# pandegroup/openmm

Hardware: NVIDIA H100
Metric: ns/day (higher is better)
Workload: dtype f32

## Files before the change

### include/b200md.h

```cpp
#ifndef B200MD_H_
#define B200MD_H_

#include <stdint.h>

#ifdef __cplusplus
extern "C" {
#endif

typedef struct b200md_ctx b200md_ctx;

#define B200MD_NB_NOCUTOFF            0
#define B200MD_NB_CUTOFF_NONPERIODIC  1
#define B200MD_NB_CUTOFF_PERIODIC     2
#define B200MD_NB_EWALD               3
#define B200MD_NB_PME                 4
#define B200MD_NB_LJPME               5

#define B200MD_TERM_BONDS      1
#define B200MD_TERM_ANGLES     2
#define B200MD_TERM_TORSIONS   4
#define B200MD_TERM_NB_DIRECT  8
#define B200MD_TERM_NB_RECIP   16
#define B200MD_TERM_RB_TORSIONS 32
#define B200MD_TERM_CMAP       64
// ... 72 lines not shown

int b200md_compute(b200md_ctx* ctx, int terms, int want_forces, double* energy);
int b200md_compute_groups(b200md_ctx* ctx, int terms, unsigned int bonded_group_mask, int want_forces, double* energy);

int b200md_set_integrator(b200md_ctx* ctx, int kind, double dt, double temperature, double friction,
                          int seed, double constraint_tol);
int b200md_step(b200md_ctx* ctx, int nsteps);
int b200md_integrate_only(b200md_ctx* ctx);
int b200md_kinetic_energy(b200md_ctx* ctx, double* ke);
int b200md_apply_constraints(b200md_ctx* ctx, double tol);
int b200md_apply_velocity_constraints(b200md_ctx* ctx, double tol);
int b200md_synchronize(b200md_ctx* ctx);

int b200md_comm_unique_id(void* id128);
int b200md_ownership_probe(int natoms, const double* mass, int ncon, const int* p1, const int* p2, const double* distance,
                           int world, int* atom_lo, int* unit_lo);
int b200md_comm_init(b200md_ctx* ctx, int rank, int world, const void* id128);

typedef struct b200md_stats {
    int64_t natoms, padded_atoms, num_blocks;
    int64_t num_tiles;
    int64_t num_mask_tiles;
    int64_t list_builds;
    int64_t force_evals;
    int64_t kernel_launches;
    int64_t pairs_in_cutoff;
    int     pme_grid[3];
    double  ewald_alpha;
    int     overflow;
    int64_t graph_instantiations;
} b200md_stats;
int b200md_get_stats(b200md_ctx* ctx, b200md_stats* out);
int b200md_time_phase(b200md_ctx* ctx, int phase, int reps, double* ms_mean);
int b200md_fft3d_r2c(int device, int nx, int ny, int nz, const float* in, float* out);
int b200md_fft3d_c2r(int device, int nx, int ny, int nz, const float* in, float* out);
void* b200md_cuda_stream(b200md_ctx* ctx);

int b200md_pme_create(b200md_ctx** out, int device, int natoms, int nx, int ny, int nz, double alpha);
int b200md_pme_exec(b200md_ctx* ctx, const float* posq, const double box[9], int include_energy, float* force4, double* energy);

#ifdef __cplusplus
}
#endif
#endif
```

### openmm_b200/_lib.py

```python
import ctypes as C
import os

_HERE = os.path.dirname(os.path.abspath(__file__))
LIB_PATH = os.environ.get("B200MD_LIB", os.path.join(_HERE, "libb200md.so"))


class NonbondedDesc(C.Structure):
    _fields_ = [("method", C.c_int), ("cutoff", C.c_double), ("use_switch", C.c_int), ("switch_distance", C.c_double),
                ("rf_dielectric", C.c_double), ("ewald_alpha", C.c_double), ("grid", C.c_int*3),
                ("dispersion_coefficient", C.c_double), ("exceptions_periodic", C.c_int)]


class Stats(C.Structure):
    _fields_ = [("natoms", C.c_int64), ("padded_atoms", C.c_int64), ("num_blocks", C.c_int64), ("num_tiles", C.c_int64),
                ("num_mask_tiles", C.c_int64), ("list_builds", C.c_int64), ("force_evals", C.c_int64),
                ("kernel_launches", C.c_int64), ("pairs_in_cutoff", C.c_int64), ("pme_grid", C.c_int*3),
                ("ewald_alpha", C.c_double), ("overflow", C.c_int),
                ("graph_instantiations", C.c_int64)]


_P = C.c_void_p
_D = C.POINTER(C.c_double)
_I = C.POINTER(C.c_int)
_F = C.POINTER(C.c_float)
# ... 23 lines not shown
    "b200md_update_nonbonded_params": (C.c_int, [_P, _D, _D, _D, C.c_int, _D, _D, _D, C.c_double]),
    "b200md_update_bonded_params": (C.c_int, [_P, C.c_int, C.c_int, _D, _D, _I]),
    "b200md_update_rb_torsion_params": (C.c_int, [_P, C.c_int, _D]),
    "b200md_update_cmap_params": (C.c_int, [_P, C.c_int, _I, _D, C.c_int, _I]),
    "b200md_set_box": (C.c_int, [_P, _D, _D, _D]),
    "b200md_get_box": (C.c_int, [_P, _D, _D, _D]),
    "b200md_set_barostat_molecules": (C.c_int, [_P, C.c_int, _I, _I]),
    "b200md_scale_coordinates": (C.c_int, [_P, C.c_double, C.c_double, C.c_double]),
    "b200md_restore_coordinates": (C.c_int, [_P]),
    "b200md_set_positions": (C.c_int, [_P, _D]),
    "b200md_get_positions": (C.c_int, [_P, _D]),
    "b200md_set_velocities": (C.c_int, [_P, _D]),
    "b200md_get_velocities": (C.c_int, [_P, _D]),
    "b200md_get_forces": (C.c_int, [_P, _D]),
    "b200md_set_time": (C.c_int, [_P, C.c_double]),
    "b200md_get_time": (C.c_double, [_P]),
    "b200md_get_step_count": (C.c_int64, [_P]),
    "b200md_checkpoint_save": (C.c_int64, [_P, _P, C.c_int64]),
    "b200md_checkpoint_load": (C.c_int, [_P, _P, C.c_int64]),
    "b200md_compute": (C.c_int, [_P, C.c_int, C.c_int, _D]),
    "b200md_compute_groups": (C.c_int, [_P, C.c_int, C.c_uint, C.c_int, _D]),
    "b200md_set_integrator": (C.c_int, [_P, C.c_int, C.c_double, C.c_double, C.c_double, C.c_int, C.c_double]),
    "b200md_step": (C.c_int, [_P, C.c_int]),
    "b200md_integrate_only": (C.c_int, [_P]),
    "b200md_kinetic_energy": (C.c_int, [_P, _D]),
    "b200md_apply_constraints": (C.c_int, [_P, C.c_double]),
    "b200md_apply_velocity_constraints": (C.c_int, [_P, C.c_double]),
    "b200md_synchronize": (C.c_int, [_P]),
    "b200md_comm_unique_id": (C.c_int, [_P]),
    "b200md_ownership_probe": (C.c_int, [C.c_int, _D, C.c_int, _I, _I, _D, C.c_int, _I, _I]),
    "b200md_comm_init": (C.c_int, [_P, C.c_int, C.c_int, _P]),
    "b200md_get_stats": (C.c_int, [_P, C.POINTER(Stats)]),
    "b200md_time_phase": (C.c_int, [_P, C.c_int, C.c_int, _D]),
    "b200md_fft3d_r2c": (C.c_int, [C.c_int, C.c_int, C.c_int, C.c_int, _F, _F]),
    "b200md_fft3d_c2r": (C.c_int, [C.c_int, C.c_int, C.c_int, C.c_int, _F, _F]),
    "b200md_pme_create": (C.c_int, [C.POINTER(_P), C.c_int, C.c_int, C.c_int, C.c_int, C.c_int, C.c_double]),
    "b200md_pme_exec": (C.c_int, [_P, _F, _D, C.c_int, _F, _D]),
    "b200md_cuda_stream": (_P, [_P]),
}

_lib = None


def load():
    global _lib
    if _lib is None:
        if not os.path.exists(LIB_PATH):
            raise RuntimeError("libb200md.so is missing (%s): build it with `python -c 'import __graft_entry__ as g; g.build()'`. "
                               "openmm_b200 has no CPU fallback." % LIB_PATH)
        lib = C.CDLL(LIB_PATH, mode=C.RTLD_GLOBAL)
        for name, (res, args) in SIGNATURES.items():
            fn = getattr(lib, name)
            fn.restype = res
            fn.argtypes = args
        _lib = lib
    return _lib
```

### openmm_b200/csrc/engine.cu

```cuda
#include "engine.h"
#include "../../include/b200md.h"
#include <stdexcept>
#include <algorithm>
#include <cmath>
#include <cstring>
#include <cstdlib>
#include <map>
#include <set>
#include <dlfcn.h>
#include <thread>

static std::string g_create_error;

template <class T> struct DevBuf {
    T* p = nullptr; size_t n = 0; bool owned = true;
    void attach(void* ptr, size_t count) { free(); p = (T*) ptr; n = count; owned = false; }
    void alloc(size_t count) {
        if (!owned) { if (count > n) throw std::runtime_error("window buffer too small"); return; }
        free(); n = count; if (count) CUDA_CHECK(cudaMalloc(&p, count*sizeof(T)));
    }
    void upload(const std::vector<T>& v) { if (v.size() > n) alloc(v.size()); if (!v.empty()) CUDA_CHECK(cudaMemcpy(p, v.data(), v.size()*sizeof(T), cudaMemcpyHostToDevice)); }
    void zero() { if (n) CUDA_CHECK(cudaMemset(p, 0, n*sizeof(T))); }
    void free() { if (p && owned) cudaFree(p); p = nullptr; n = 0; owned = true; }
    ~DevBuf() { free(); }
// ... 308 lines not shown
}

static void cell_order(const int nc[3], std::vector<int>& rank) {
    const int sx = (nc[0] + 1)/2, sy = (nc[1] + 1)/2, sz = (nc[2] + 1)/2;
    rank.assign((size_t) nc[0]*nc[1]*nc[2], 0);
    int r = 0;
    for (int ix = 0; ix < sx; ix++)
        for (int jy = 0; jy < sy; jy++) {
            const int iy = (ix & 1) ? sy-1-jy : jy;
            for (int kz = 0; kz < sz; kz++) {
                const int iz = ((ix*sy + jy) & 1) ? sz-1-kz : kz;
                for (int a = 0; a < 2; a++) for (int b = 0; b < 2; b++) for (int c = 0; c < 2; c++) {
                    const int x = 2*ix + a, y = 2*iy + b, z = 2*iz + c;
                    if (x < nc[0] && y < nc[1] && z < nc[2]) rank[((size_t) x*nc[1] + y)*nc[2] + z] = r++;
                }
            }
        }
}

static void setup_cells(b200md_ctx* c) {
    int nc[3] = {1, 1, 1};
    if (c->nb.box.periodic) {
        const double vol = c->boxA[0]*c->boxB[1]*c->boxC[2];
        const double density = c->natoms/vol;
        double edge = std::cbrt(4.0/density);
        const double L[3] = {c->boxA[0], c->boxB[1], c->boxC[2]};
        for (int d = 0; d < 3; d++) nc[d] = std::max(1, std::min(128, (int) std::floor(L[d]/edge)));
    }
    const int ncells = nc[0]*nc[1]*nc[2];
    if (ncells != c->nb.ncells || nc[0] != c->nb.ncell[0] || nc[1] != c->nb.ncell[1] || nc[2] != c->nb.ncell[2]) {
        std::vector<int> rank;
        cell_order(nc, rank);
        c->cellRank.upload(rank);
        c->cellCount.alloc(ncells + 1); c->cellCount.zero();
        c->cellFill.alloc(ncells); c->cellFill.zero();
        c->nb.ncells = ncells;
        for (int d = 0; d < 3; d++) c->nb.ncell[d] = nc[d];
        c->nb.cellRank = c->cellRank.p; c->nb.cellCount = c->cellCount.p; c->nb.cellFill = c->cellFill.p;
    }
}

static void invalidate_graph(b200md_ctx* c) { c->graphValid = false; c->multiValid = false; }

static void apply_box(b200md_ctx* c) {
    BoxDev& b = c->nb.box;
    const int m = c->nbdesc.method;
    b.periodic = (m == B200MD_NB_CUTOFF_PERIODIC || m == B200MD_NB_PME) ? 1 : 0;
    if (c->haveBox) {
        b.ax = (float) c->boxA[0]; b.bx = (float) c->boxB[0]; b.by = (float) c->boxB[1];
        b.cx = (float) c->boxC[0]; b.cy = (float) c->boxC[1]; b.cz = (float) c->boxC[2];
        b.invAx = (float) (1.0/c->boxA[0]); b.invBy = (float) (1.0/c->boxB[1]); b.invCz = (float) (1.0/c->boxC[2]);
        b.dax = c->boxA[0]; b.dby = c->boxB[1]; b.dcz = c->boxC[2];
        b.triclinic = (c->boxB[0] != 0 || c->boxC[0] != 0 || c->boxC[1] != 0) ? 1 : 0;
        const double det = c->boxA[0]*c->boxB[1]*c->boxC[2];
        const double s = 1.0/det;
        double* R = b.recip;
        R[0] = c->boxB[1]*c->boxC[2]*s; R[1] = 0; R[2] = 0;
        R[3] = -c->boxB[0]*c->boxC[2]*s; R[4] = c->boxA[0]*c->boxC[2]*s; R[5] = 0;
        R[6] = (c->boxB[0]*c->boxC[1] - c->boxB[1]*c->boxC[0])*s; R[7] = -c->boxA[0]*c->boxC[1]*s; R[8] = c->boxA[0]*c->boxB[1]*s;
        b.volume = det;
    }
    else {
        require(!b.periodic, "periodic nonbonded method needs box vectors (b200md_set_box)");
        b.ax = b.by = b.cz = 1.f; b.bx = b.cx = b.cy = 0.f; b.invAx = b.invBy = b.invCz = 1.f; b.triclinic = 0; b.dax = b.dby = b.dcz = 1;
        for (int i = 0; i < 9; i++) b.recip[i] = 0; b.volume = 1;
    }
    if (b.periodic) {
// ... 1417 lines not shown
    c->forceEvals++;
    c->hforce.resize((size_t) 3*c->npad);
    double he[B200MD_NUM_ENERGY] = {0};
    CUDA_CHECK(cudaMemcpyAsync(c->hforce.data(), c->force.p, sizeof(long long)*3*c->npad, cudaMemcpyDeviceToHost, c->stream));
    if (include_energy) CUDA_CHECK(cudaMemcpyAsync(he, c->energy.p, sizeof(he), cudaMemcpyDeviceToHost, c->stream));
    CUDA_CHECK(cudaStreamSynchronize(c->stream));
    const double s = 1.0/B200MD_FORCE_SCALE;
    for (int i = 0; i < c->natoms; i++)
        for (int k = 0; k < 3; k++) force4[4*i+k] = (float) (s*(double) c->hforce[(size_t) k*c->npad + i]);
    if (energy) *energy = include_energy ? he[EN_RECIP] : 0.0;
    API_END(ctx)
}

extern "C" int b200md_get_stats(b200md_ctx* ctx, b200md_stats* out) {
    API_BEGIN(ctx)
    memset(out, 0, sizeof(*out));
    out->natoms = ctx->natoms; out->padded_atoms = ctx->npad; out->num_blocks = ctx->nblocks;
    if (ctx->finalized) {
        launch_count_pairs(ctx->nb, ctx->stream);
        int h[16], lc[2*LC_STRIDE];
        CUDA_CHECK(cudaMemcpyAsync(h, ctx->counters.p, sizeof(int)*16, cudaMemcpyDeviceToHost, ctx->stream));
        CUDA_CHECK(cudaMemcpyAsync(lc, ctx->listCounters.p, sizeof(lc), cudaMemcpyDeviceToHost, ctx->stream));
        CUDA_CHECK(cudaStreamSynchronize(ctx->stream));
        const int* cur = lc + LC_STRIDE*(h[CT_CUR] & 1);
        int masks = 0;
        for (int r = 0; r < TILE_REGIONS; r++) masks += cur[LC_MASKS + r];
        out->num_tiles = cur[LC_USED]; out->num_mask_tiles = masks; out->overflow = h[CT_OVERFLOW]; out->list_builds = h[CT_BUILDS]; out->pairs_in_cutoff = h[CT_PAIRS];
    }
    out->force_evals = ctx->forceEvals; out->kernel_launches = ctx->kernelLaunches; out->graph_instantiations = ctx->graphInstantiations;
    out->pme_grid[0] = ctx->pme.nx; out->pme_grid[1] = ctx->pme.ny; out->pme_grid[2] = ctx->pme.nz; out->ewald_alpha = ctx->pme.alpha;
    API_END(ctx)
}

extern "C" int b200md_time_phase(b200md_ctx* ctx, int phase, int reps, double* ms_mean) {
    API_BEGIN(ctx)
    require(ctx->finalized, "time_phase before finalize");
    b200md_ctx* c = ctx;
    prepare_list(c);
    c->stepStateValid = false;
    cudaStream_t s = c->stream;
    const NbDev nbv = role_nb(c);
    CommDev local{}; local.world = 1;
    cudaEvent_t e0, e1;
    CUDA_CHECK(cudaEventCreate(&e0)); CUDA_CHECK(cudaEventCreate(&e1));
    const int one = 1;
    double total = 0;
    DevBuf<float4> savePos, saveVel, saveCorr; DevBuf<double4> saveVelD; unsigned long long saveStep = 0;
    auto restoreState = [&]() {
        CUDA_CHECK(cudaMemcpyAsync(c->posq.p, savePos.p, sizeof(float4)*c->npad, cudaMemcpyDeviceToDevice, s));
        CUDA_CHECK(cudaMemcpyAsync(c->velm.p, saveVel.p, sizeof(float4)*c->npad, cudaMemcpyDeviceToDevice, s));
        if (c->mixed()) {
            CUDA_CHECK(cudaMemcpyAsync(c->posqCorr.p, saveCorr.p, sizeof(float4)*c->npad, cudaMemcpyDeviceToDevice, s));
            CUDA_CHECK(cudaMemcpyAsync(c->velmD.p, saveVelD.p, sizeof(double4)*c->npad, cudaMemcpyDeviceToDevice, s));
        }
    };
    if (phase == 4) {
        require(c->haveIntegrator, "time_phase(integrate) before set_integrator");
        savePos.alloc(c->npad); saveVel.alloc(c->npad);
        CUDA_CHECK(cudaMemcpyAsync(savePos.p, c->posq.p, sizeof(float4)*c->npad, cudaMemcpyDeviceToDevice, s));
        CUDA_CHECK(cudaMemcpyAsync(saveVel.p, c->velm.p, sizeof(float4)*c->npad, cudaMemcpyDeviceToDevice, s));
        if (c->mixed()) {
            saveCorr.alloc(c->npad); saveVelD.alloc(c->npad);
            CUDA_CHECK(cudaMemcpyAsync(saveCorr.p, c->posqCorr.p, sizeof(float4)*c->npad, cudaMemcpyDeviceToDevice, s));
            CUDA_CHECK(cudaMemcpyAsync(saveVelD.p, c->velmD.p, sizeof(double4)*c->npad, cudaMemcpyDeviceToDevice, s));
        }
        CUDA_CHECK(cudaMemcpyAsync(&saveStep, c->stepCounter.p, sizeof(saveStep), cudaMemcpyDeviceToHost, s));
// ... 70 lines not shown
```

### openmm_b200/csrc/engine.h

```cpp
#pragma once
#include <cuda_runtime.h>
#include <stdint.h>
#include <stdexcept>
#include <string>
#include <vector>

#define B200MD_TILE 32
#define B200MD_PME_ORDER 5
#define B200MD_FORCE_SCALE 4294967296.0
#define B200MD_ONE_4PI_EPS0 138.93545764438198
#define B200MD_BOLTZ 0.00831446261815324
#define B200MD_MAX_RADIX 16
#define B200MD_MAX_FFT_STAGES 8

#define CUDA_CHECK(x) do { cudaError_t e_ = (x); if (e_ != cudaSuccess) throw std::runtime_error(std::string(#x) + ": " + cudaGetErrorString(e_)); } while (0)

template <typename... P, typename... A>
inline void launch_high(void (*kernel)(P...), dim3 grid, dim3 block, size_t smem, cudaStream_t s, A... args) {
    static const int hi = [] { int lo = 0, h = 0; cudaDeviceGetStreamPriorityRange(&lo, &h); return h; }();
    cudaLaunchAttribute at[1];
    at[0].id = cudaLaunchAttributePriority;
    at[0].val.priority = hi;
    cudaLaunchConfig_t cfg = {};
    cfg.gridDim = grid; cfg.blockDim = block; cfg.dynamicSmemBytes = smem; cfg.stream = s;
// ... 16 lines not shown
typedef double2 real2;
#else
typedef float real;
typedef float2 real2;
#endif

struct FftPlanDev {
    int n;
    int nstages;
    int radix[B200MD_MAX_FFT_STAGES];
    const real2* tw;
};

struct ListDev {
    float4* sposq;
    float2* ssigeps;
    float4* swrap;
    int* sorig;
    float4* blockCenter;
    float4* blockHalf;
    float4* superCenter;
    float4* superHalf;
    int* tileI;
    int* tileJ;
    int* tileMask;
    unsigned int* maskPool;
    int* lc;
};
#define TILE_REGIONS 32
enum { LC_TILES = 0, LC_MASKS = TILE_REGIONS, LC_MAXHALF = 2*TILE_REGIONS, LC_USED = 2*TILE_REGIONS + 1, LC_STRIDE = 128 };

enum { CT_PAIRSTART = 0,
       CT_REBUILD = 2, CT_OVERFLOW = 3, CT_BUILDS = 4, CT_PAIRS = 5, CT_CUR = 10, CT_CURSOR = 14,
       CT_BTDONE = 7, CT_BAR = 9, CT_BAREXIT = 15 };

struct NbDev {
    BoxDev box;
    int natoms, npad, nblocks;
    int method;
    int useSwitch;
    float cutoff, cutoff2, paddedCutoff2, switchDist;
    float alpha;
    float krf, crf;
    float dispDummy;
    float4* posq;
    float4* velm;
    float4* posqCorr;
    double4* velmD;
    float2* sigeps;
    const double* chargeD;
    const double2* sigepsD;
    long long* force;
    double* energy;
    ListDev list[2];
    int* sortedOf;
    float4* refPos;
    int ncell[3];
    int ncells;
    const int* cellRank;
    int* cellCount;
    int* cellFill;
    int* atomCell;
    int* tmpSorted;
    float4* atomShift;
    int maxTiles;
    int* counters;
    const int* exclStart;
// ... 306 lines not shown
```

### openmm_b200/csrc/nonbonded.cu

```cuda
#include "engine.h"
#include "../../include/b200md.h"
#include <algorithm>

#define FULL 0xffffffffu

__device__ __forceinline__ float3 min_image(float3 d, const BoxDev& b) {
    if (b.triclinic) {
        float s = floorf(d.z*b.invCz + 0.5f);
        d.x -= s*b.cx; d.y -= s*b.cy; d.z -= s*b.cz;
        s = floorf(d.y*b.invBy + 0.5f);
        d.x -= s*b.bx; d.y -= s*b.by;
        s = floorf(d.x*b.invAx + 0.5f);
        d.x -= s*b.ax;
    }
    else {
        d.x -= b.ax*rintf(d.x*b.invAx);
        d.y -= b.by*rintf(d.y*b.invBy);
        d.z -= b.cz*rintf(d.z*b.invCz);
    }
    return d;
}

__device__ __forceinline__ float box_dist2(float3 d, float hx, float hy, float hz, const BoxDev& b, bool periodic) {
    if (periodic) d = min_image(d, b);
    if (!periodic || !b.triclinic) {
        const float dx = fmaxf(0.f, fabsf(d.x) - hx), dy = fmaxf(0.f, fabsf(d.y) - hy), dz = fmaxf(0.f, fabsf(d.z) - hz);
        return dx*dx + dy*dy + dz*dz;
    }
    float best = 3e38f;
    for (int sz = -1; sz <= 1; sz++)
        for (int sy = -1; sy <= 1; sy++)
            for (int sx = -1; sx <= 1; sx++) {
                const float x = d.x + sx*b.ax + sy*b.bx + sz*b.cx;
                const float y = d.y + sy*b.by + sz*b.cy;
                const float z = d.z + sz*b.cz;
                const float dx = fmaxf(0.f, fabsf(x) - hx), dy = fmaxf(0.f, fabsf(y) - hy), dz = fmaxf(0.f, fabsf(z) - hz);
                best = fminf(best, dx*dx + dy*dy + dz*dz);
            }
    return best;
}

__global__ void __launch_bounds__(256) k_check_gather(NbDev nb, CommDev cd) {
    comm_wait(cd, CH_POS, cd.world > 1 ? *cd.posNeed : 0ull);
    const int s = blockIdx.x*blockDim.x + threadIdx.x;
    const ListDev& L = nb.list[nb.counters[CT_CUR] & 1];
    if (s == 0) { nb.counters[CT_CURSOR] = 0; nb.counters[CT_PAIRSTART] = 0; }
    if (s < nb.natoms) {
        const float4 p = nb.posq[s];
        const float4 r = nb.refPos[s];
        const float dx = p.x-r.x, dy = p.y-r.y, dz = p.z-r.z;
        const float d2 = dx*dx + dy*dy + dz*dz;
        if (!(d2 <= nb.halfPad2))
            nb.counters[CT_REBUILD] = 1;
    }
    if (s < nb.npad) {
        int a = L.sorig[s];
        if (a < 0 || a >= nb.natoms) a = L.sorig[nb.natoms-1];
        a = min(max(a, 0), nb.natoms-1);
        float4 p = nb.posq[a];
        if (s >= nb.natoms) p.w = 0.f;
        L.sposq[s] = p;
    }
}

__device__ __forceinline__ void wrap_molecule(const NbDev& nb, int m) {
    const int begin = nb.molStart[m], end = nb.molStart[m+1];
    const float4 p = nb.posq[nb.molAtoms[begin]];
    const double* R = nb.box.recip;
    const double px = p.x - nb.origin[0], py = p.y - nb.origin[1], pz = p.z - nb.origin[2];
    const double f[3] = {px*R[0] + py*R[3] + pz*R[6], px*R[1] + py*R[4] + pz*R[7], px*R[2] + py*R[5] + pz*R[8]};
    int k[3];
    bool move = false;
    for (int d = 0; d < 3; d++) {
        const double w = floor(f[d]);
        k[d] = (w >= 2.0 || w <= -2.0) ? (int) w : 0;
        move |= (k[d] != 0);
    }
    if (!move) return;
    const BoxDev& b = nb.box;
    const double sx = -(k[0]*(double) b.dax + k[1]*(double) b.bx + k[2]*(double) b.cx);
    const double sy = -(k[1]*(double) b.dby + k[2]*(double) b.cy);
    const double sz = -(k[2]*(double) b.dcz);
    for (int t = begin; t < end; t++) {
        const int a = nb.molAtoms[t];
        if (nb.posqCorr) {
            const double4 q = load_pos<double>(nb, a);
            store_pos<double>(nb, a, q.x + sx, q.y + sy, q.z + sz);
        }
        else {
            const float4 q = nb.posq[a];
            nb.posq[a] = make_float4((float) ((double) q.x + sx), (float) ((double) q.y + sy), (float) ((double) q.z + sz), q.w);
        }
        nb.cellOffset[a] += k[0]; nb.cellOffset[a + nb.npad] += k[1]; nb.cellOffset[a + 2*nb.npad] += k[2];
    }
}

__device__ __forceinline__ void bin_atom(const NbDev& nb, int a) {
    float4 p = nb.posq[a];
    int key = 0;
    float4 shift = make_float4(0, 0, 0, 0);
    if (nb.box.periodic) {
        const double* R = nb.box.recip;
        double f[3];
        const double px = p.x - nb.origin[0], py = p.y - nb.origin[1], pz = p.z - nb.origin[2];
        f[0] = px*R[0] + py*R[3] + pz*R[6];
        f[1] = px*R[1] + py*R[4] + pz*R[7];
        f[2] = px*R[2] + py*R[5] + pz*R[8];
        int c[3];
        float fl[3];
        for (int d = 0; d < 3; d++) {
            double w = floor(f[d]);
            fl[d] = (float) w;
            double fr = f[d] - w;
            int ci = (int) (fr*nb.ncell[d]);
            c[d] = min(max(ci, 0), nb.ncell[d]-1);
        }
        shift.x = -(fl[0]*nb.box.ax + fl[1]*nb.box.bx + fl[2]*nb.box.cx);
        shift.y = -(fl[1]*nb.box.by + fl[2]*nb.box.cy);
        shift.z = -(fl[2]*nb.box.cz);
        key = nb.cellRank[(c[0]*nb.ncell[1] + c[1])*nb.ncell[2] + c[2]];
    }
    else
        key = 0;
    nb.atomCell[a] = key;
    nb.atomShift[a] = shift;
    atomicAdd(&nb.cellCount[key], 1);
}

__device__ void scan_cells_block(const NbDev& nb, int* partial) {
    int n = nb.ncells;
    int per = (n + blockDim.x - 1)/blockDim.x;
    int begin = threadIdx.x*per, end = min(begin+per, n);
    int sum = 0;
    for (int i = begin; i < end; i++) sum += nb.cellCount[i];
    partial[threadIdx.x] = sum;
    __syncthreads();
    for (int off = 1; off < blockDim.x; off <<= 1) {
        int v = (threadIdx.x >= off) ? partial[threadIdx.x-off] : 0;
        __syncthreads();
        partial[threadIdx.x] += v;
        __syncthreads();
    }
    int run = partial[threadIdx.x] - sum;
    for (int i = begin; i < end; i++) {
        int c = nb.cellCount[i];
        nb.cellCount[i] = run;
        run += c;
    }
    if (threadIdx.x == 0) nb.cellCount[n] = nb.natoms;
}

__device__ __forceinline__ void fill_atom(const NbDev& nb, int a) {
    int key = nb.atomCell[a];
    int slot = nb.cellCount[key] + atomicAdd(&nb.cellFill[key], 1);
    nb.tmpSorted[slot] = a;
}

__device__ __forceinline__ void finalize_slot(const NbDev& nb, const ListDev& L, int s) {
    if (s < nb.natoms) {
        int a = s;
        if (nb.box.periodic) {
            a = nb.tmpSorted[s];
            const int key = nb.atomCell[a];
            const int begin = nb.cellCount[key], end = nb.cellCount[key+1];
            int rank = 0;
            for (int t = begin; t < end; t++) rank += (nb.tmpSorted[t] < a);
            s = begin + rank;
        }
        float4 p = nb.posq[a];
        float4 sh = nb.atomShift[a];
        L.sorig[s] = a;
        nb.sortedOf[a] = s;
        L.swrap[s] = make_float4(p.x+sh.x, p.y+sh.y, p.z+sh.z, p.w);
        L.sposq[s] = p;
        L.ssigeps[s] = nb.sigeps[a];
        nb.refPos[a] = p;
        if (s == 0) L.lc[LC_MAXHALF] = 0;
    }
    else {
        L.sorig[s] = -1;
        L.ssigeps[s] = make_float2(0, 0);
    }
}

__device__ __forceinline__ void grid_barrier(const NbDev& nb, int target) {
    __syncthreads();
    if (threadIdx.x == 0) {
        __threadfence();
        atomicAdd(&nb.counters[CT_BAR], 1);
        long spins = 0;
        while (*((volatile int*) &nb.counters[CT_BAR]) < target) {
            __nanosleep(32);
            if (++spins > (1L << 23)) { nb.counters[CT_OVERFLOW] = 2; break; }
        }
        __threadfence();
    }
    __syncthreads();
}

__device__ void list_prep_phases(const NbDev& nb, const ListDev& L, int* partial) {
    const int G = gridDim.x;
    const int gtid = blockIdx.x*blockDim.x + threadIdx.x, gthreads = G*blockDim.x;
    const int lane = threadIdx.x & 31, gwarp = gtid >> 5, gwarps = gthreads >> 5;
    int base = 0;
    if (nb.nmol > 0) {
        for (int m = gtid; m < nb.nmol; m += gthreads) wrap_molecule(nb, m);
        grid_barrier(nb, G);
        base = G;
    }
    for (int a = gtid; a < nb.natoms; a += gthreads) bin_atom(nb, a);
    grid_barrier(nb, base + G);
    if (blockIdx.x == 0) scan_cells_block(nb, partial);
    grid_barrier(nb, base + 2*G);
    for (int a = gtid; a < nb.natoms; a += gthreads) fill_atom(nb, a);
    grid_barrier(nb, base + 3*G);
    for (int s = gtid; s < nb.npad; s += gthreads) finalize_slot(nb, L, s);
    grid_barrier(nb, base + 4*G);
    for (int b = gwarp; b < nb.nblocks; b += gwarps) {
        const int s = b*32 + lane;
        const int sl = min(s, nb.natoms-1);
        const float4 p = L.swrap[sl];
        if (s >= nb.natoms) { L.swrap[s] = make_float4(p.x, p.y, p.z, 0.f); L.sposq[s] = make_float4(p.x, p.y, p.z, 0.f); }
        float lox = p.x, hix = p.x, loy = p.y, hiy = p.y, loz = p.z, hiz = p.z;
        for (int off = 16; off > 0; off >>= 1) {
            lox = fminf(lox, __shfl_xor_sync(FULL, lox, off)); hix = fmaxf(hix, __shfl_xor_sync(FULL, hix, off));
            loy = fminf(loy, __shfl_xor_sync(FULL, loy, off)); hiy = fmaxf(hiy, __shfl_xor_sync(FULL, hiy, off));
            loz = fminf(loz, __shfl_xor_sync(FULL, loz, off)); hiz = fmaxf(hiz, __shfl_xor_sync(FULL, hiz, off));
        }
        if (lane == 0) {
            L.blockCenter[b] = make_float4(0.5f*(lox+hix), 0.5f*(loy+hiy), 0.5f*(loz+hiz), 0);
            L.blockHalf[b] = make_float4(0.5f*(hix-lox), 0.5f*(hiy-loy), 0.5f*(hiz-loz), 0);
            atomicMax(&L.lc[LC_MAXHALF], __float_as_int(0.5f*fmaxf(hix-lox, fmaxf(hiy-loy, hiz-loz))));
        }
    }
    for (int i = gtid; i <= nb.ncells; i += gthreads) {
        nb.cellCount[i] = 0;
        if (i < nb.ncells) nb.cellFill[i] = 0;
    }
    if (gtid < TILE_REGIONS) { L.lc[LC_TILES + gtid] = 0; L.lc[LC_MASKS + gtid] = 0; }
    grid_barrier(nb, base + 5*G);
    const int nsuper = (nb.nblocks + 31) >> 5;
    for (int sb = gwarp; sb < nsuper; sb += gwarps) {
        const int b = sb*32 + lane;
        float lox = 3e38f, hix = -3e38f, loy = 3e38f, hiy = -3e38f, loz = 3e38f, hiz = -3e38f;
        if (b < nb.nblocks) {
            const float4 c = L.blockCenter[b], h = L.blockHalf[b];
            lox = c.x - h.x; hix = c.x + h.x; loy = c.y - h.y; hiy = c.y + h.y; loz = c.z - h.z; hiz = c.z + h.z;
        }
        for (int off = 16; off > 0; off >>= 1) {
            lox = fminf(lox, __shfl_xor_sync(FULL, lox, off)); hix = fmaxf(hix, __shfl_xor_sync(FULL, hix, off));
            loy = fminf(loy, __shfl_xor_sync(FULL, loy, off)); hiy = fmaxf(hiy, __shfl_xor_sync(FULL, hiy, off));
            loz = fminf(loz, __shfl_xor_sync(FULL, loz, off)); hiz = fmaxf(hiz, __shfl_xor_sync(FULL, hiz, off));
        }
        if (lane == 0) {
            L.superCenter[sb] = make_float4(0.5f*(lox+hix), 0.5f*(loy+hiy), 0.5f*(loz+hiz), 0);
            L.superHalf[sb] = make_float4(0.5f*(hix-lox), 0.5f*(hiy-loy), 0.5f*(hiz-loz), 0);
        }
    }
}
__device__ __forceinline__ void grid_barrier_exit(const NbDev& nb) {
    __syncthreads();
    if (threadIdx.x == 0) {
        __threadfence();
        if (atomicAdd(&nb.counters[CT_BAREXIT], 1) == (int) gridDim.x - 1) { nb.counters[CT_BAR] = 0; nb.counters[CT_BAREXIT] = 0; }
    }
}

__global__ void __launch_bounds__(256) k_list_prep(NbDev nb) {
    if (nb.counters[CT_REBUILD] == 0) return;
    const ListDev& L = nb.list[(nb.counters[CT_CUR] & 1) ^ 1];
    __shared__ int partial[256];
    list_prep_phases(nb, L, partial);
    grid_barrier_exit(nb);
}

#define MAX_CACHED_EXCL 24
#define SB_MAX 1024
__device__ void flush_tile(const NbDev& nb, const ListDev& L, int ib, const int* buf, int count, bool diagonal, int lane,
                           const int* sexc, int nexc, int e0) {
    const int region = ib % TILE_REGIONS;
    const int cap = nb.maxTiles/TILE_REGIONS;
    int k = 0;
    if (lane == 0) k = atomicAdd(&L.lc[LC_TILES + region], 1);
    k = __shfl_sync(FULL, k, 0);
    if (k >= cap) { if (lane == 0) nb.counters[CT_OVERFLOW] = 1; return; }
    const int t = region*cap + k;
    int myj = (lane < count) ? buf[lane] : -1;
    L.tileJ[t*32 + lane] = myj;
    unsigned int valid = (count >= 32) ? FULL : ((1u << count) - 1u);
    unsigned int mask = valid;
    bool need = (count < 32);
    int si = ib*32 + lane;
    if (diagonal) {
        unsigned int le = (lane == 31) ? FULL : ((2u << lane) - 1u);
        mask &= ~le;
        need = true;
    }
    if (si >= nb.natoms) { mask = 0; need = true; }
    else {
        const int jlo = buf[0], jhi = buf[count-1];
        for (int e = 0; e < nexc; e++) {
            const int sj = (e < MAX_CACHED_EXCL) ? sexc[e] : nb.sortedOf[nb.exclList[e0 + e]];
            if (sj < jlo || sj > jhi) continue;
            int lo = 0, hi = count-1;
            while (lo < hi) { int mid = (lo+hi) >> 1; if (buf[mid] < sj) lo = mid+1; else hi = mid; }
// ... 190 lines not shown
            }
        }
    }
    }
    if (exactCull && nstg > 0) exact_stage(nstg);
    if (lane == 0) S.sleft[w] = nbuf;
    group_sync(barId, NW*32);
    int total = 0;
    for (int q = 0; q < NW; q++) total += S.sleft[q];
    if (lane < nbuf) {
        const int v = buf[lane];
        int rank = 0;
        for (int q = 0; q < NW; q++) {
            const int nq = S.sleft[q];
            for (int k = 0; k < nq; k++) rank += (S.sbuf[q][k] < v);
        }
        S.smerged[rank] = v;
    }
    group_sync(barId, NW*32);
    for (int off = 32*w; off < total; off += 32*NW)
        flush_tile(nb, L, ib, S.smerged + off, min(32, total - off), false, lane, sexc, nexc, e0);
    group_sync(barId, NW*32);
}

template <int NW>
__global__ void __launch_bounds__(NW*32, 40/NW) k_build_tiles(NbDev nb) {
    if (nb.counters[CT_REBUILD] == 0) return;
    if (nb.world > 1 && ((int) blockIdx.x % nb.world) != nb.rank) {
        if (threadIdx.x == 0) list_block_done(nb);
        return;
    }
    const ListDev& L = nb.list[(nb.counters[CT_CUR] & 1) ^ 1];
    __shared__ BuildSmem<NW> S;
    build_tiles_iblock<NW>(nb, L, blockIdx.x, threadIdx.x >> 5, threadIdx.x & 31, S, 1);
    if (threadIdx.x == 0) list_block_done(nb);
}

void launch_check_displacement(const NbDev& nb, const CommDev& cd, cudaStream_t s) {
    k_check_gather<<<(nb.npad+255)/256, 256, 0, s>>>(nb, cd);
}

void launch_list_build(const NbDev& nb, cudaStream_t s) {
    int dev = 0, sms = 132;
    cudaGetDevice(&dev);
    cudaDeviceGetAttribute(&sms, cudaDevAttrMultiProcessorCount, dev);
    k_list_prep<<<std::max(1, std::min((nb.npad + 255)/256, 2*sms)), 256, 0, s>>>(nb);
    if (nb.nblocks <= 1200) k_build_tiles<8><<<nb.nblocks, 256, 0, s>>>(nb);
    else k_build_tiles<4><<<nb.nblocks, 128, 0, s>>>(nb);
}

#define PME_G_WMAX 14.0f

__device__ __forceinline__ float rcp_approx(float x) { float r; asm("rcp.approx.ftz.f32 %0, %1;" : "=f"(r) : "f"(x)); return r; }
__device__ __forceinline__ float rsqrt_approx(float x) { float r; asm("rsqrt.approx.ftz.f32 %0, %1;" : "=f"(r) : "f"(x)); return r; }

__device__ __forceinline__ float ewald_g(float w) {
    const float p = fmaf(w, fmaf(w, fmaf(w, fmaf(w, fmaf(w, -3.521083106e-07f, 3.445905357e-05f), 0.0002032837893f), 0.01676110697f), -0.01832553619f), 0.7522528288f);
    const float q = fmaf(w, fmaf(w, fmaf(w, fmaf(w, fmaf(w, 0.0001580620439f, 0.002480551583f), 0.02451798422f), 0.1533710339f), 0.5756407144f), 1.0f);
    return p*rcp_approx(q);
}

struct TileCursor {
    int incl, total, cap;
    __device__ __forceinline__ void init(const NbDev& nb, const ListDev& L, int lane) {
        cap = nb.maxTiles/TILE_REGIONS;
        int c = min(L.lc[LC_TILES + lane], cap);
        for (int off = 1; off < 32; off <<= 1) {
            const int v = __shfl_up_sync(FULL, c, off);
            if (lane >= off) c += v;
        }
        incl = c;
        total = __shfl_sync(FULL, c, 31);
    }
    __device__ __forceinline__ int slot(int f) const {
        const int r = __popc(__ballot_sync(FULL, incl <= f));
        const int before = __shfl_sync(FULL, incl, max(r-1, 0));
        return r*cap + f - (r > 0 ? before : 0);
    }
};
// ... 371 lines not shown
```

### openmm_b200/engine.py

```python
import ctypes as C
import numpy as np
from . import _lib
from .systems import SystemDesc, NB_PME

TERM_BONDS, TERM_ANGLES, TERM_TORSIONS, TERM_NB_DIRECT, TERM_NB_RECIP = 1, 2, 4, 8, 16
TERM_RB_TORSIONS, TERM_CMAP, TERM_ALL = 32, 64, 127
BONDED_KINDS = {"bonds": 0, "angles": 1, "torsions": 2, "rb_torsions": 3, "cmap": 4}
PHASES = {"pair": 0, "pme_spread": 1, "pme_fft_conv": 2, "pme_gather": 3, "integrate": 4, "list_build": 5, "bonded": 6}


class EngineError(RuntimeError):
    pass


def _dp(a):
    return a.ctypes.data_as(C.POINTER(C.c_double))


def _ip(a):
    return a.ctypes.data_as(C.POINTER(C.c_int))


def _f64(a):
    return np.ascontiguousarray(a, dtype=np.float64)
# ... 166 lines not shown
    def apply_constraints(self, tol=1e-5):
        self._ck(self.lib.b200md_apply_constraints(self.h, tol))

    def apply_velocity_constraints(self, tol=1e-5):
        self._ck(self.lib.b200md_apply_velocity_constraints(self.h, tol))

    def synchronize(self):
        self._ck(self.lib.b200md_synchronize(self.h))

    def time(self):
        return self.lib.b200md_get_time(self.h)

    def checkpoint(self):
        n = self.lib.b200md_checkpoint_save(self.h, None, 0)
        buf = C.create_string_buffer(n)
        if self.lib.b200md_checkpoint_save(self.h, C.cast(buf, C.c_void_p), n) != n:
            raise EngineError(self.lib.b200md_last_error(self.h).decode())
        return buf.raw

    def load_checkpoint(self, blob):
        buf = C.create_string_buffer(blob, len(blob))
        self._ck(self.lib.b200md_checkpoint_load(self.h, C.cast(buf, C.c_void_p), len(blob)))

    def stats(self):
        s = _lib.Stats()
        self._ck(self.lib.b200md_get_stats(self.h, C.byref(s)))
        return {k: (list(getattr(s, k)) if k == "pme_grid" else getattr(s, k)) for k, _ in s._fields_}

    def time_phase(self, phase, reps=20):
        ms = C.c_double()
        self._ck(self.lib.b200md_time_phase(self.h, PHASES[phase] if isinstance(phase, str) else phase, reps, C.byref(ms)))
        return ms.value

    def stream(self):
        return self.lib.b200md_cuda_stream(self.h)

    def close(self):
        if getattr(self, "h", None):
            self.lib.b200md_destroy(self.h)
            self.h = None

    def __del__(self):
        try:
            self.close()
        except Exception:
            pass


def fft3d_r2c(x, device=0):
    lib = _lib.load()
    x = np.ascontiguousarray(x, dtype=np.float32)
    nx, ny, nz = x.shape
    out = np.empty((nx, ny, nz//2+1, 2), dtype=np.float32)
    fp = C.POINTER(C.c_float)
    if lib.b200md_fft3d_r2c(device, nx, ny, nz, x.ctypes.data_as(fp), out.ctypes.data_as(fp)) != 0:
        raise EngineError(lib.b200md_last_error(None).decode())
    return out[..., 0] + 1j*out[..., 1]


def fft3d_c2r(c, nz, device=0):
    lib = _lib.load()
    nx, ny, nzc = c.shape
    assert nzc == nz//2+1
    inp = np.ascontiguousarray(np.stack([c.real, c.imag], -1), dtype=np.float32)
    out = np.empty((nx, ny, nz), dtype=np.float32)
    fp = C.POINTER(C.c_float)
# ... 4 lines not shown
```

Baseline: 1315.

## Parallelize cell-count scan across CTAs and skip molecule wrapping when unneeded

The cell prefix scan in list prep moves from a single-block serial scan to a chunked multi-CTA scan: each block scans its chunk with warp shuffles and stores a chunk total, and every block then scans the chunk totals into shared memory to get its offsets. Molecule wrapping in list prep now runs only when the displacement-check kernel has set a wrap flag because some molecule drifted two or more box lengths. The aim is to cut the serial scan and the per-rebuild wrap pass out of neighbour-list rebuilds. It also adds a list-snapshot debug API and optional timing stamps, and caps the prep grid at 512 CTAs.

```diff
diff --git a/include/b200md.h b/include/b200md.h
--- a/include/b200md.h
+++ b/include/b200md.h
@@ -128,6 +128,7 @@
 } b200md_stats;
 int b200md_get_stats(b200md_ctx* ctx, b200md_stats* out);
 int b200md_time_phase(b200md_ctx* ctx, int phase, int reps, double* ms_mean);
+int64_t b200md_get_list(b200md_ctx* ctx, int* sorig, int* rows, int64_t max_rows);
 int b200md_fft3d_r2c(int device, int nx, int ny, int nz, const float* in, float* out);
 int b200md_fft3d_c2r(int device, int nx, int ny, int nz, const float* in, float* out);
 void* b200md_cuda_stream(b200md_ctx* ctx);
diff --git a/openmm_b200/_lib.py b/openmm_b200/_lib.py
--- a/openmm_b200/_lib.py
+++ b/openmm_b200/_lib.py
@@ -79,6 +79,7 @@
     "b200md_comm_init": (C.c_int, [_P, C.c_int, C.c_int, _P]),
     "b200md_get_stats": (C.c_int, [_P, C.POINTER(Stats)]),
     "b200md_time_phase": (C.c_int, [_P, C.c_int, C.c_int, _D]),
+    "b200md_get_list": (C.c_int64, [_P, _I, _I, C.c_int64]),
     "b200md_fft3d_r2c": (C.c_int, [C.c_int, C.c_int, C.c_int, C.c_int, _F, _F]),
     "b200md_fft3d_c2r": (C.c_int, [C.c_int, C.c_int, C.c_int, C.c_int, _F, _F]),
     "b200md_pme_create": (C.c_int, [C.POINTER(_P), C.c_int, C.c_int, C.c_int, C.c_int, C.c_int, C.c_double]),
diff --git a/openmm_b200/csrc/engine.cu b/openmm_b200/csrc/engine.cu
--- a/openmm_b200/csrc/engine.cu
+++ b/openmm_b200/csrc/engine.cu
@@ -364,7 +364,7 @@
         std::vector<int> rank;
         cell_order(nc, rank);
         c->cellRank.upload(rank);
-        c->cellCount.alloc(ncells + 1); c->cellCount.zero();
+        c->cellCount.alloc(ncells + 1 + PREP_MAX_CTAS); c->cellCount.zero();
         c->cellFill.alloc(ncells); c->cellFill.zero();
         c->nb.ncells = ncells;
         for (int d = 0; d < 3; d++) c->nb.ncell[d] = nc[d];
@@ -1848,6 +1848,46 @@
     API_END(ctx)
 }
 
+extern "C" int64_t b200md_get_list(b200md_ctx* ctx, int* sorig, int* rows, int64_t max_rows) {
+    if (!ctx) return -1;
+    try {
+        CUDA_CHECK(cudaSetDevice(ctx->device));
+        require(ctx->finalized && ctx->haveNb, "get_list needs a finalized context with a nonbonded force");
+        prepare_list(ctx);
+        int h[16], lc[2*LC_STRIDE];
+        CUDA_CHECK(cudaMemcpyAsync(h, ctx->counters.p, sizeof(h), cudaMemcpyDeviceToHost, ctx->stream));
+        CUDA_CHECK(cudaMemcpyAsync(lc, ctx->listCounters.p, sizeof(lc), cudaMemcpyDeviceToHost, ctx->stream));
+        CUDA_CHECK(cudaStreamSynchronize(ctx->stream));
+        const int l = h[CT_CUR] & 1;
+        const int* cnt = lc + LC_STRIDE*l;
+        const int cap = ctx->nb.maxTiles/TILE_REGIONS;
+        int64_t ntiles = 0;
+        for (int r = 0; r < TILE_REGIONS; r++) ntiles += std::min(cnt[LC_TILES + r], cap);
+        if (!rows) return ntiles;
+        require(max_rows >= ntiles, "get_list: rows holds fewer than num_tiles rows");
+        const size_t T = ctx->nb.maxTiles;
+        std::vector<int> ti(T), tm(T), tj(T*32);
+        std::vector<unsigned int> mp(T*32);
+        CUDA_CHECK(cudaMemcpy(sorig, ctx->sorig[l].p, sizeof(int)*ctx->npad, cudaMemcpyDeviceToHost));
+        CUDA_CHECK(cudaMemcpy(ti.data(), ctx->tileI[l].p, sizeof(int)*T, cudaMemcpyDeviceToHost));
+        CUDA_CHECK(cudaMemcpy(tm.data(), ctx->tileMask[l].p, sizeof(int)*T, cudaMemcpyDeviceToHost));
+        CUDA_CHECK(cudaMemcpy(tj.data(), ctx->tileJ[l].p, sizeof(int)*T*32, cudaMemcpyDeviceToHost));
+        CUDA_CHECK(cudaMemcpy(mp.data(), ctx->maskPool[l].p, sizeof(unsigned int)*T*32, cudaMemcpyDeviceToHost));
+        int* row = rows;
+        for (int r = 0; r < TILE_REGIONS; r++)
+            for (int k = 0; k < std::min(cnt[LC_TILES + r], cap); k++, row += 66) {
+                const size_t t = (size_t) r*cap + k;
+                row[0] = ti[t];
+                row[1] = tm[t] >= 0;
+                for (int q = 0; q < 32; q++) {
+                    row[2 + q] = tj[t*32 + q];
+                    row[34 + q] = tm[t] >= 0 ? (int) mp[(size_t) tm[t]*32 + q] : -1;
+                }
+            }
+        return ntiles;
+    } catch (std::exception& e) { ctx->err = e.what(); return -1; }
+}
+
 extern "C" int b200md_time_phase(b200md_ctx* ctx, int phase, int reps, double* ms_mean) {
     API_BEGIN(ctx)
     require(ctx->finalized, "time_phase before finalize");
diff --git a/openmm_b200/csrc/engine.h b/openmm_b200/csrc/engine.h
--- a/openmm_b200/csrc/engine.h
+++ b/openmm_b200/csrc/engine.h
@@ -72,7 +72,9 @@
 
 enum { CT_PAIRSTART = 0,
        CT_REBUILD = 2, CT_OVERFLOW = 3, CT_BUILDS = 4, CT_PAIRS = 5, CT_CUR = 10, CT_CURSOR = 14,
-       CT_BTDONE = 7, CT_BAR = 9, CT_BAREXIT = 15 };
+       CT_BTDONE = 7, CT_BAR = 9, CT_BAREXIT = 15,
+       CT_WRAP = 8 };
+const int PREP_MAX_CTAS = 512;
 
 struct NbDev {
     BoxDev box;
diff --git a/openmm_b200/csrc/nonbonded.cu b/openmm_b200/csrc/nonbonded.cu
--- a/openmm_b200/csrc/nonbonded.cu
+++ b/openmm_b200/csrc/nonbonded.cu
@@ -38,6 +38,20 @@
                 best = fminf(best, dx*dx + dy*dy + dz*dz);
             }
     return best;
+}
+
+__device__ __forceinline__ bool wrap_lattice_shift(const NbDev& nb, float4 p, int* k) {
+    const double* R = nb.box.recip;
+    const double px = p.x - nb.origin[0], py = p.y - nb.origin[1], pz = p.z - nb.origin[2];
+    const double f[3] = {px*R[0] + py*R[3] + pz*R[6], px*R[1] + py*R[4] + pz*R[7], px*R[2] + py*R[5] + pz*R[8]};
+    bool move = false;
+    for (int d = 0; d < 3; d++) {
+        const double w = floor(f[d]);
+        const int kd = (w >= 2.0 || w <= -2.0) ? (int) w : 0;
+        if (k) k[d] = kd;
+        move |= (kd != 0);
+    }
+    return move;
 }
 
 __global__ void __launch_bounds__(256) k_check_gather(NbDev nb, CommDev cd) {
@@ -52,6 +66,7 @@
         const float d2 = dx*dx + dy*dy + dz*dz;
         if (!(d2 <= nb.halfPad2))
             nb.counters[CT_REBUILD] = 1;
+        if (nb.nmol > 0 && wrap_lattice_shift(nb, p, nullptr)) nb.counters[CT_WRAP] = 1;
     }
     if (s < nb.npad) {
         int a = L.sorig[s];
@@ -65,18 +80,8 @@
 
 __device__ __forceinline__ void wrap_molecule(const NbDev& nb, int m) {
     const int begin = nb.molStart[m], end = nb.molStart[m+1];
-    const float4 p = nb.posq[nb.molAtoms[begin]];
-    const double* R = nb.box.recip;
-    const double px = p.x - nb.origin[0], py = p.y - nb.origin[1], pz = p.z - nb.origin[2];
-    const double f[3] = {px*R[0] + py*R[3] + pz*R[6], px*R[1] + py*R[4] + pz*R[7], px*R[2] + py*R[5] + pz*R[8]};
     int k[3];
-    bool move = false;
-    for (int d = 0; d < 3; d++) {
-        const double w = floor(f[d]);
-        k[d] = (w >= 2.0 || w <= -2.0) ? (int) w : 0;
-        move |= (k[d] != 0);
-    }
-    if (!move) return;
+    if (!wrap_lattice_shift(nb, nb.posq[nb.molAtoms[begin]], k)) return;
     const BoxDev& b = nb.box;
     const double sx = -(k[0]*(double) b.dax + k[1]*(double) b.bx + k[2]*(double) b.cx);
     const double sy = -(k[1]*(double) b.dby + k[2]*(double) b.cy);
@@ -127,42 +132,72 @@
     atomicAdd(&nb.cellCount[key], 1);
 }
 
-__device__ void scan_cells_block(const NbDev& nb, int* partial) {
-    int n = nb.ncells;
-    int per = (n + blockDim.x - 1)/blockDim.x;
-    int begin = threadIdx.x*per, end = min(begin+per, n);
+__device__ __forceinline__ int block_scan(int v, int* warpSums, int* total) {
+    const int lane = threadIdx.x & 31, warp = threadIdx.x >> 5;
+    for (int off = 1; off < 32; off <<= 1) {
+        const int u = __shfl_up_sync(FULL, v, off);
+        if (lane >= off) v += u;
+    }
+    if (lane == 31) warpSums[warp] = v;
+    __syncthreads();
+    int before = 0, sum = 0;
+    for (int q = 0; q < (int) (blockDim.x >> 5); q++) {
+        const int s = warpSums[q];
+        before += (q < warp) ? s : 0;
+        sum += s;
+    }
+    __syncthreads();
+    *total = sum;
+    return v + before;
+}
+
+__device__ void scan_cells_chunk(const NbDev& nb, int* warpSums) {
+    const int cs = (nb.ncells + gridDim.x - 1)/gridDim.x;
+    const int begin = blockIdx.x*cs, end = min(begin + cs, nb.ncells);
+    int carry = 0;
+    for (int base = begin; base < end; base += blockDim.x) {
+        const int i = base + threadIdx.x;
+        const int v = (i < end) ? nb.cellCount[i] : 0;
+        int total;
+        const int incl = block_scan(v, warpSums, &total);
+        if (i < end) nb.cellCount[i] = carry + incl - v;
+        carry += total;
+    }
+    if (threadIdx.x == 0) nb.cellCount[nb.ncells + 1 + blockIdx.x] = carry;
+}
+
+__device__ void scan_chunk_totals(const NbDev& nb, int* chunkStart, int* warpSums) {
+    const int G = gridDim.x;
+    const int per = (G + blockDim.x - 1)/blockDim.x;
+    const int b0 = threadIdx.x*per;
     int sum = 0;
-    for (int i = begin; i < end; i++) sum += nb.cellCount[i];
-    partial[threadIdx.x] = sum;
+    for (int k = 0; k < per; k++) sum += (b0 + k < G) ? nb.cellCount[nb.ncells + 1 + b0 + k] : 0;
+    int total;
+    int run = block_scan(sum, warpSums, &total) - sum;
+    for (int k = 0; k < per; k++)
+        if (b0 + k < G) { chunkStart[b0 + k] = run; run += nb.cellCount[nb.ncells + 1 + b0 + k]; }
     __syncthreads();
-    for (int off = 1; off < blockDim.x; off <<= 1) {
-        int v = (threadIdx.x >= off) ? partial[threadIdx.x-off] : 0;
-        __syncthreads();
-        partial[threadIdx.x] += v;
-        __syncthreads();
-    }
-    int run = partial[threadIdx.x] - sum;
-    for (int i = begin; i < end; i++) {
-        int c = nb.cellCount[i];
-        nb.cellCount[i] = run;
-        run += c;
-    }
-    if (threadIdx.x == 0) nb.cellCount[n] = nb.natoms;
-}
-
-__device__ __forceinline__ void fill_atom(const NbDev& nb, int a) {
+}
+
+__device__ __forceinline__ int cell_start(const NbDev& nb, const int* chunkStart, int key) {
+    if (key >= nb.ncells) return nb.natoms;
+    const int cs = (nb.ncells + gridDim.x - 1)/gridDim.x;
+    return chunkStart[key/cs] + nb.cellCount[key];
+}
+
+__device__ __forceinline__ void fill_atom(const NbDev& nb, const int* chunkStart, int a) {
     int key = nb.atomCell[a];
-    int slot = nb.cellCount[key] + atomicAdd(&nb.cellFill[key], 1);
+    int slot = cell_start(nb, chunkStart, key) + atomicAdd(&nb.cellFill[key], 1);
     nb.tmpSorted[slot] = a;
 }
 
-__device__ __forceinline__ void finalize_slot(const NbDev& nb, const ListDev& L, int s) {
+__device__ __forceinline__ void finalize_slot(const NbDev& nb, const ListDev& L, const int* chunkStart, int s) {
     if (s < nb.natoms) {
         int a = s;
         if (nb.box.periodic) {
             a = nb.tmpSorted[s];
             const int key = nb.atomCell[a];
-            const int begin = nb.cellCount[key], end = nb.cellCount[key+1];
+            const int begin = cell_start(nb, chunkStart, key), end = cell_start(nb, chunkStart, key + 1);
             int rank = 0;
             for (int t = begin; t < end; t++) rank += (nb.tmpSorted[t] < a);
             s = begin + rank;
@@ -198,24 +233,45 @@
     __syncthreads();
 }
 
-__device__ void list_prep_phases(const NbDev& nb, const ListDev& L, int* partial) {
+#ifdef B200MD_LIST_STAMPS
+__device__ unsigned long long g_listStamps[16];
+__device__ __forceinline__ unsigned long long global_ns() { unsigned long long t; asm volatile("mov.u64 %0, %%globaltimer;" : "=l"(t)); return t; }
+#define LIST_STAMP(k) if (blockIdx.x == 0 && threadIdx.x == 0) { const unsigned long long t = global_ns(); g_listStamps[k] += t - tstamp; tstamp = t; }
+extern "C" int b200md_list_stamps(unsigned long long* out) {
+    return cudaMemcpyFromSymbol(out, g_listStamps, sizeof(g_listStamps)) == cudaSuccess ? 0 : -1;
+}
+#else
+#define LIST_STAMP(k)
+#endif
+
+__device__ void list_prep_phases(const NbDev& nb, const ListDev& L, int* chunkStart, int* warpSums) {
     const int G = gridDim.x;
     const int gtid = blockIdx.x*blockDim.x + threadIdx.x, gthreads = G*blockDim.x;
     const int lane = threadIdx.x & 31, gwarp = gtid >> 5, gwarps = gthreads >> 5;
+#ifdef B200MD_LIST_STAMPS
+    unsigned long long tstamp = global_ns();
+    if (blockIdx.x == 0 && threadIdx.x == 0) g_listStamps[7] += 1;
+#endif
     int base = 0;
-    if (nb.nmol > 0) {
+    if (nb.nmol > 0 && nb.counters[CT_WRAP]) {
         for (int m = gtid; m < nb.nmol; m += gthreads) wrap_molecule(nb, m);
         grid_barrier(nb, G);
         base = G;
     }
+    LIST_STAMP(0)
     for (int a = gtid; a < nb.natoms; a += gthreads) bin_atom(nb, a);
     grid_barrier(nb, base + G);
-    if (blockIdx.x == 0) scan_cells_block(nb, partial);
+    LIST_STAMP(1)
+    scan_cells_chunk(nb, warpSums);
     grid_barrier(nb, base + 2*G);
-    for (int a = gtid; a < nb.natoms; a += gthreads) fill_atom(nb, a);
+    scan_chunk_totals(nb, chunkStart, warpSums);
+    LIST_STAMP(2)
+    for (int a = gtid; a < nb.natoms; a += gthreads) fill_atom(nb, chunkStart, a);
     grid_barrier(nb, base + 3*G);
-    for (int s = gtid; s < nb.npad; s += gthreads) finalize_slot(nb, L, s);
+    LIST_STAMP(3)
+    for (int s = gtid; s < nb.npad; s += gthreads) finalize_slot(nb, L, chunkStart, s);
     grid_barrier(nb, base + 4*G);
+    LIST_STAMP(4)
     for (int b = gwarp; b < nb.nblocks; b += gwarps) {
         const int s = b*32 + lane;
         const int sl = min(s, nb.natoms-1);
@@ -239,6 +295,7 @@
     }
     if (gtid < TILE_REGIONS) { L.lc[LC_TILES + gtid] = 0; L.lc[LC_MASKS + gtid] = 0; }
     grid_barrier(nb, base + 5*G);
+    LIST_STAMP(5)
     const int nsuper = (nb.nblocks + 31) >> 5;
     for (int sb = gwarp; sb < nsuper; sb += gwarps) {
         const int b = sb*32 + lane;
@@ -257,20 +314,27 @@
             L.superHalf[sb] = make_float4(0.5f*(hix-lox), 0.5f*(hiy-loy), 0.5f*(hiz-loz), 0);
         }
     }
+#ifdef B200MD_LIST_STAMPS
+    __syncthreads();
+#endif
+    LIST_STAMP(6)
 }
 __device__ __forceinline__ void grid_barrier_exit(const NbDev& nb) {
     __syncthreads();
     if (threadIdx.x == 0) {
         __threadfence();
-        if (atomicAdd(&nb.counters[CT_BAREXIT], 1) == (int) gridDim.x - 1) { nb.counters[CT_BAR] = 0; nb.counters[CT_BAREXIT] = 0; }
+        if (atomicAdd(&nb.counters[CT_BAREXIT], 1) == (int) gridDim.x - 1) {
+            nb.counters[CT_BAR] = 0; nb.counters[CT_BAREXIT] = 0; nb.counters[CT_WRAP] = 0;
+        }
     }
 }
 
 __global__ void __launch_bounds__(256) k_list_prep(NbDev nb) {
     if (nb.counters[CT_REBUILD] == 0) return;
     const ListDev& L = nb.list[(nb.counters[CT_CUR] & 1) ^ 1];
-    __shared__ int partial[256];
-    list_prep_phases(nb, L, partial);
+    __shared__ int chunkStart[PREP_MAX_CTAS];
+    __shared__ int warpSums[8];
+    list_prep_phases(nb, L, chunkStart, warpSums);
     grid_barrier_exit(nb);
 }
 
@@ -527,7 +591,16 @@
     }
     const ListDev& L = nb.list[(nb.counters[CT_CUR] & 1) ^ 1];
     __shared__ BuildSmem<NW> S;
+#ifdef B200MD_LIST_STAMPS
+    const unsigned long long t0 = global_ns();
+#endif
     build_tiles_iblock<NW>(nb, L, blockIdx.x, threadIdx.x >> 5, threadIdx.x & 31, S, 1);
+#ifdef B200MD_LIST_STAMPS
+    if (threadIdx.x == 0) {
+        const unsigned long long span = global_ns() - t0;
+        atomicAdd(&g_listStamps[8], span); atomicAdd(&g_listStamps[9], 1ull); atomicMax(&g_listStamps[10], span);
+    }
+#endif
     if (threadIdx.x == 0) list_block_done(nb);
 }
 
@@ -539,7 +612,7 @@
     int dev = 0, sms = 132;
     cudaGetDevice(&dev);
     cudaDeviceGetAttribute(&sms, cudaDevAttrMultiProcessorCount, dev);
-    k_list_prep<<<std::max(1, std::min((nb.npad + 255)/256, 2*sms)), 256, 0, s>>>(nb);
+    k_list_prep<<<std::max(1, std::min({(nb.npad + 255)/256, 2*sms, PREP_MAX_CTAS})), 256, 0, s>>>(nb);
     if (nb.nblocks <= 1200) k_build_tiles<8><<<nb.nblocks, 256, 0, s>>>(nb);
     else k_build_tiles<4><<<nb.nblocks, 128, 0, s>>>(nb);
 }
diff --git a/openmm_b200/engine.py b/openmm_b200/engine.py
--- a/openmm_b200/engine.py
+++ b/openmm_b200/engine.py
@@ -222,6 +222,16 @@
         self._ck(self.lib.b200md_time_phase(self.h, PHASES[phase] if isinstance(phase, str) else phase, reps, C.byref(ms)))
         return ms.value
 
+    def list_snapshot(self):
+        n = self.lib.b200md_get_list(self.h, None, None, 0)
+        if n < 0:
+            raise EngineError(self.lib.b200md_last_error(self.h).decode())
+        sorig = np.empty(self.stats()["padded_atoms"], dtype=np.int32)
+        rows = np.empty((max(n, 1), 66), dtype=np.int32)
+        if self.lib.b200md_get_list(self.h, _ip(sorig), _ip(rows), len(rows)) != n:
+            raise EngineError(self.lib.b200md_last_error(self.h).decode())
+        return sorig, rows[:n]
+
     def stream(self):
         return self.lib.b200md_cuda_stream(self.h)
 
```

Result: no change. 1325 (median of 6 runs) (+0.8%).
